# Netflix/metaflow

Hardware: AMD Instinct MI355X
Metric: tokens/sec (higher is better)
Workload: dtype bf16; 1 GPU; model=llama3-8b, global_batch=8, seq_len=4096, parallelism=dp1

## Files before the change

metaflow_amd/ops/csrc/attention.hip:

```cpp

#include "common.h"

#define ATT_D 128

typedef __attribute__((ext_vector_type(16))) float f16f;

DEV f16f mfma32(bf16x8 a, bf16x8 b, f16f c) {
  return __builtin_amdgcn_mfma_f32_32x32x16_bf16(a, b, c, 0, 0, 0);
}

struct WaveCoord {
  int wid, lane, l32, hi;
};

DEV WaveCoord wave_coord() {
  WaveCoord c;
  c.wid = threadIdx.x / WAVE;
  c.lane = threadIdx.x & (WAVE - 1);
  c.l32 = c.lane & 31;
  c.hi = c.lane >> 5;
  return c;
}

DEV int c_row(int r, int hi) { return (r & 3) + 8 * (r >> 2) + 4 * hi; }

DEV unsigned int pack_bf2(float lo, float hi) {
  union { __hip_bfloat162 h; unsigned int u; } c;
  c.h = __float22bfloat162_rn(make_float2(lo, hi));
  return c.u;
}

template <int NT>
DEV void col_to_afrags(const f16f* st, bf16x8* pa, int hi) {
  unsigned int pk[NT * 8], xp[NT * 8];
#pragma unroll
  for (int t = 0; t < NT; ++t)
#pragma unroll
    for (int j2 = 0; j2 < 8; ++j2)
      pk[t * 8 + j2] = pack_bf2(st[t][j2 * 2], st[t][j2 * 2 + 1]);
#pragma unroll
  for (int i = 0; i < NT * 8; ++i) xp[i] = __shfl_xor(pk[i], 32, WAVE);
#pragma unroll
  for (int ks = 0; ks < NT * 2; ++ks) {
    union {
      unsigned int w[4];
      bf16x8 v;
    } u;
    if (hi == 0) {
      u.w[0] = pk[4 * ks];
      u.w[1] = pk[4 * ks + 1];
      u.w[2] = xp[4 * ks];
      u.w[3] = xp[4 * ks + 1];
    } else {
      u.w[0] = xp[4 * ks + 2];
      u.w[1] = xp[4 * ks + 3];
      u.w[2] = pk[4 * ks + 2];
      u.w[3] = pk[4 * ks + 3];
    }
    pa[ks] = u.v;
  }
}


template <int ROWS, int BLOCK>
DEV void stage_panel(short* dst, const short* src,
                     long long src_row_stride) {
  constexpr int TOT = ROWS * 16;
#pragma unroll
  for (int it = 0; it < (TOT + BLOCK - 1) / BLOCK; ++it) {
    const int idx = it * BLOCK + threadIdx.x;
    if (idx < TOT) {
      const int r = idx % ROWS, c8 = idx / ROWS;
      bf16x8 v = *(const bf16x8*)(src + r * src_row_stride + c8 * 8);
      *(bf16x8*)(dst + (c8 >> 1) * (ROWS * 16) + r * 16 + (c8 & 1) * 8) =
          v;
    }
  }
}

template <int ROWS>
DEV bf16x8 frag8_panel(const short* tile, int row, int d0) {
  return *(const bf16x8*)(tile + (d0 >> 4) * (ROWS * 16) + row * 16
                          + (d0 & 15));
}

DEV unsigned long long tr_read(const short* lds_ptr) {
  unsigned int addr = (unsigned int)(unsigned long long)lds_ptr;
  unsigned long long out;
  asm volatile("ds_read_b64_tr_b16 %0, %1" : "=v"(out) : "v"(addr));
  return out;
}

union BFrag {
  unsigned long long u[2];
  bf16x8 v;
};

template <int ROWS>
DEV void tr_load_bfrags(BFrag bfr[4], const short* tile, int row0,
                        int lane, int hi) {
  const int tr_lane_off = (((lane >> 2) & 3) * 16) + (lane & 3) * 4;
  const int tr_panel = ((lane >> 4) & 1) * (ROWS * 16);
#pragma unroll
  for (int n = 0; n < 4; ++n) {
    const int base = n * 2 * (ROWS * 16) + tr_panel
                     + (row0 + hi * 8) * 16 + tr_lane_off;
    bfr[n].u[0] = tr_read(tile + base);
    bfr[n].u[1] = tr_read(tile + base + 4 * 16);
  }
}

DEV void put_elem(short* p, float x) { *p = f2bf(x); }
DEV void put_elem(float* p, float x) { *p = x; }

template <bool ROW_SCALE, typename T>
DEV void store_acc_tile(T* dst, long long off0, int row0, const f16f acc[4],
                        int l32, int hi, float lane_scale = 1.f) {
#pragma unroll
  for (int r = 0; r < 16; ++r) {
    const int row_local = c_row(r, hi);
    float f = 1.f;
    if (ROW_SCALE) f = __shfl(lane_scale, row_local + 32 * hi, WAVE);
    const long long obase = off0 + (long long)(row0 + row_local) * ATT_D;
#pragma unroll
    for (int n = 0; n < 4; ++n)
      put_elem(dst + obase + n * 32 + l32,
               ROW_SCALE ? acc[n][r] * f : acc[n][r]);
  }
}

DEV void acc_to_bfrags(const f16f& x, bf16x8* pb) {
#pragma unroll
  for (int s = 0; s < 2; ++s) {
    unsigned int w[4];
#pragma unroll
    for (int i = 0; i < 4; ++i)
      w[i] = pack_bf2(x[8 * s + 2 * i], x[8 * s + 2 * i + 1]);
    union {
      unsigned int w[4];
      bf16x8 v;
    } u;
#pragma unroll
    for (int i = 0; i < 2; ++i) {
      auto r = __builtin_amdgcn_permlane32_swap(w[i], w[2 + i], false,
                                                false);
      u.w[i] = r[0];
      u.w[2 + i] = r[1];
    }
    pb[s] = u.v;
  }
}

DEV float half_pair_max(float x) {
  const unsigned int u = __float_as_uint(x);
  auto r = __builtin_amdgcn_permlane32_swap(u, u, false, false);
  return fmaxf(__uint_as_float(r[0]), __uint_as_float(r[1]));
}

DEV float half_pair_sum(float x) {
  const unsigned int u = __float_as_uint(x);
  auto r = __builtin_amdgcn_permlane32_swap(u, u, false, false);
  return __uint_as_float(r[0]) + __uint_as_float(r[1]);
}

DEV void lds_wave_fence() {
  __builtin_amdgcn_fence(__ATOMIC_RELEASE, "wavefront");
  __builtin_amdgcn_wave_barrier();
  __builtin_amdgcn_fence(__ATOMIC_ACQUIRE, "wavefront");
}

template <int NB, bool ROW_SCALE>
DEV void store_acc_tile_t_bf16(short* dst, long long off0, short* tw,
                               const f16f acc[4], int lane,
                               float lane_scale = 1.f) {
  constexpr int SLOTS = NB * 4;
  constexpr int ROWLEN = NB * 32;
  const int l32 = lane & 31, hi = lane >> 5;
#pragma unroll
  for (int p = 0; p < 4 / NB; ++p) {
#pragma unroll
    for (int nb = 0; nb < NB; ++nb) {
      const int n = p * NB + nb;
#pragma unroll
      for (int g = 0; g < 4; ++g) {
        bf16x4 w;
#pragma unroll
        for (int j = 0; j < 4; ++j)
          w[j] = f2bf(ROW_SCALE ? acc[n][4 * g + j] * lane_scale
                                : acc[n][4 * g + j]);
        const int slot = (nb * 4 + g) ^ (l32 & (SLOTS - 1));
        *(bf16x4*)(tw + l32 * ROWLEN + slot * 8 + hi * 4) = w;
      }
    }
    lds_wave_fence();
#pragma unroll
    for (int i = 0; i < SLOTS / 2; ++i) {
      const int row = i * (64 / SLOTS) + lane / SLOTS;
      const int c = lane & (SLOTS - 1);
      const bf16x8 v = *(const bf16x8*)(tw + row * ROWLEN
                                        + ((c ^ (row & (SLOTS - 1))) * 8));
      *(bf16x8*)(dst + off0 + (long long)row * ATT_D + p * ROWLEN + c * 8) =
          v;
    }
    if (p + 1 < 4 / NB) lds_wave_fence();
  }
}

struct BlockCoord {
  int rank, h, b;
};

DEV BlockCoord block_coord(int T, int H) {
  const int bid = blockIdx.x;
  const int per_b = T * H;
  BlockCoord c;
  c.b = bid / per_b;
  const int r = bid - c.b * per_b;
  c.rank = r / H;
  c.h = r - c.rank * H;
  return c;
}


template <int BLOCK>
__global__ __launch_bounds__(512) void attn_fwd_v2_kernel(
    const short* __restrict__ q, const short* __restrict__ k,
    const short* __restrict__ v, short* __restrict__ o,
    float* __restrict__ lse, int B, int H, int Hkv, int S, float scale,
    int causal) {
  constexpr int BQ = 256, BKV = 64;
  __shared__ short kp[2][BKV * ATT_D];
  __shared__ short vp[2][BKV * ATT_D];

  const BlockCoord bc = block_coord(S / BQ, H);
  const int qb = S / BQ - 1 - bc.rank;
  const int h = bc.h;
  const int b = bc.b;
  const int hk = h / (H / Hkv);
  const WaveCoord c = wave_coord();
  const int wid = c.wid, lane = c.lane, l32 = c.l32, hi = c.hi;

  const int my_qrow = qb * BQ + wid * 32 + l32;
  const long long hoff = ((long long)b * H + h) * S;
  const long long qoff = (hoff + qb * BQ) * ATT_D;
  const long long kvoff0 = ((long long)b * Hkv + hk) * S * ATT_D;

  bf16x8 q_reg[8];
  {
    const short* qrow = q + (hoff + my_qrow) * ATT_D;
#pragma unroll
    for (int s = 0; s < 8; ++s)
      q_reg[s] = *(const bf16x8*)(qrow + s * 16 + hi * 8);
  }

  float m_run = -INFINITY;
  float l_run = 0.f;
  f16f acc_o[4];
#pragma unroll
  for (int n = 0; n < 4; ++n) acc_o[n] = (f16f){};

  const int tid = threadIdx.x;
  bf16x8 stg_k[2], stg_v[2];
  int stg_r[2], stg_c8[2];
#pragma unroll
  for (int u = 0; u < 2; ++u) {
    const int idx = u * BLOCK + tid;
    stg_r[u] = idx / 16;
    stg_c8[u] = idx % 16;
  }

#define MFX_STAGE_LOAD(jj)                                               \
  {                                                                      \
    const short* kb_ = k + kvoff0 + (long long)(jj) * BKV * ATT_D;       \
    const short* vb_ = v + kvoff0 + (long long)(jj) * BKV * ATT_D;       \
    _Pragma("unroll") for (int u = 0; u < 2; ++u) {                      \
      stg_k[u] = *(const bf16x8*)(kb_ + stg_r[u] * ATT_D + stg_c8[u] * 8);\
      stg_v[u] = *(const bf16x8*)(vb_ + stg_r[u] * ATT_D + stg_c8[u] * 8);\
    }                                                                    \
  }

#define MFX_STAGE_WRITE(buf)                                             \
  {                                                                      \
    _Pragma("unroll") for (int u = 0; u < 2; ++u) {                      \
      const int pel_ = (stg_c8[u] >> 1) * (BKV * 16) + stg_r[u] * 16     \
                       + (stg_c8[u] & 1) * 8;                            \
      *(bf16x8*)(kp[buf] + pel_) = stg_k[u];                             \
      *(bf16x8*)(vp[buf] + pel_) = stg_v[u];                             \
    }                                                                    \
  }

  const int kv_tiles =
      causal ? (qb * BQ + BQ) / BKV : S / BKV;
  MFX_STAGE_LOAD(0);
  MFX_STAGE_WRITE(0);
  __syncthreads();
  for (int j = 0; j < kv_tiles; ++j) {
    const int cur = j & 1;
    if (j + 1 < kv_tiles) MFX_STAGE_LOAD(j + 1);

    const bool active = !causal || (j * BKV <= qb * BQ + wid * 32 + 31);
    if (active) {

    f16f st[2];
#pragma unroll
    for (int t = 0; t < 2; ++t) {
      st[t] = (f16f){};
#pragma unroll
      for (int s = 0; s < 8; ++s) {
        bf16x8 kf = frag8_panel<BKV>(kp[cur], t * 32 + l32,
                                     s * 16 + hi * 8);
        st[t] = mfma32(kf, q_reg[s], st[t]);
      }
    }

    const bool diag = causal && (j * BKV + BKV > qb * BQ);
    float pmax = -INFINITY;
#pragma unroll
    for (int t = 0; t < 2; ++t) {
#pragma unroll
      for (int r = 0; r < 16; ++r) {
        float sv = st[t][r] * scale;
        if (diag) {
          const int kvg = j * BKV + t * 32 + c_row(r, hi);
          if (kvg > my_qrow) sv = -INFINITY;
        }
        st[t][r] = sv;
        pmax = fmaxf(pmax, sv);
      }
    }
    pmax = half_pair_max(pmax);
    const float newm = fmaxf(m_run, pmax);
    const float rescale = __expf(m_run - newm);
    m_run = newm;

    float psum = 0.f;
#pragma unroll
    for (int t = 0; t < 2; ++t)
#pragma unroll
      for (int r = 0; r < 16; ++r) {
        float e = __expf(st[t][r] - newm);
        st[t][r] = e;
        psum += e;
      }
    psum = half_pair_sum(psum);
    l_run = l_run * rescale + psum;

#pragma unroll
    for (int n = 0; n < 4; ++n)
#pragma unroll
      for (int r = 0; r < 16; ++r) acc_o[n][r] *= rescale;

    bf16x8 pb[4];
    acc_to_bfrags(st[0], pb);
    acc_to_bfrags(st[1], pb + 2);

    {
      const int tr_lane_off = (((lane >> 2) & 3) * 16) + (lane & 3) * 4;
      const int tr_panel = ((lane >> 4) & 1) * (BKV * 16);
#pragma unroll
      for (int ks = 0; ks < 4; ++ks) {
        BFrag bfr[4];
#pragma unroll
        for (int n = 0; n < 4; ++n) {
          const int base = n * 2 * (BKV * 16) + tr_panel
                           + (ks * 16 + hi * 8) * 16 + tr_lane_off;
          bfr[n].u[0] = tr_read(vp[cur] + base);
          bfr[n].u[1] = tr_read(vp[cur] + base + 4 * 16);
        }
        asm volatile("s_waitcnt lgkmcnt(0)");
        __builtin_amdgcn_sched_barrier(0);
#pragma unroll
        for (int n = 0; n < 4; ++n)
          acc_o[n] = mfma32(bfr[n].v, pb[ks], acc_o[n]);
      }
    }
    }

    if (j + 1 < kv_tiles) MFX_STAGE_WRITE(cur ^ 1);
    __syncthreads();
  }
#undef MFX_STAGE_LOAD
#undef MFX_STAGE_WRITE

  float inv_l = 1.f / l_run;
  short* tw = (wid < 4 ? &kp[0][0] : &vp[0][0]) + (wid & 3) * (32 * ATT_D);
  store_acc_tile_t_bf16<4, true>(o, qoff + (long long)wid * 32 * ATT_D, tw,
                                 acc_o, lane, inv_l);
  if (hi == 0)
    lse[hoff + my_qrow] = m_run + __logf(l_run);
}

__global__ void attn_bwd_delta_kernel(const short* __restrict__ dout,
                                      const short* __restrict__ o,
                                      float* __restrict__ delta,
                                      long long rows) {
  const int lane = threadIdx.x & (WAVE - 1);
  const int wid = threadIdx.x / WAVE;
  const long long row = (long long)blockIdx.x * (blockDim.x / WAVE) + wid;
  if (row >= rows) return;
  const short* dr = dout + row * ATT_D;
  const short* orow = o + row * ATT_D;
  float s = bf2f(dr[lane]) * bf2f(orow[lane])
            + bf2f(dr[lane + 64]) * bf2f(orow[lane + 64]);
  s = wave_sum(s);
  if (lane == 0) delta[row] = s;
}


extern __shared__ __attribute__((aligned(16))) short dq_kv2[];
#define DQ_DYN_LDS (2 * 64 * ATT_D * 2)

template <int BLOCK>
__global__ __launch_bounds__(512) void attn_bwd_dq_v2_kernel(
    const short* __restrict__ q, const short* __restrict__ k,
    const short* __restrict__ v, const short* __restrict__ dout,
    const float* __restrict__ lse, const float* __restrict__ delta,
    short* __restrict__ dq, int B, int H, int Hkv, int S, float scale,
    int causal) {
  constexpr int BQ = 256, BKV = 64;
  __shared__ short kp[BKV * ATT_D];
  __shared__ short vp[BKV * ATT_D];

  const BlockCoord bc = block_coord(S / BQ, H);
  const int qb = S / BQ - 1 - bc.rank;
  const int h = bc.h;
  const int b = bc.b;
  const int hk = h / (H / Hkv);
  const int wid = threadIdx.x / WAVE;
  const int lane = threadIdx.x & (WAVE - 1);
  const int l32 = lane & 31;
  const int hi = lane >> 5;

  const int my_qrow = qb * BQ + wid * 32 + l32;
  const long long hoff = ((long long)b * H + h) * S;
  const long long qoff = (hoff + qb * BQ) * ATT_D;
  const long long kvoff0 = ((long long)b * Hkv + hk) * S * ATT_D;

  bf16x8 q_reg[8], do_reg[8];
  {
    const short* qrow = q + (hoff + my_qrow) * ATT_D;
    const short* drow = dout + (hoff + my_qrow) * ATT_D;
#pragma unroll
    for (int s = 0; s < 8; ++s) {
      q_reg[s] = *(const bf16x8*)(qrow + s * 16 + hi * 8);
      do_reg[s] = *(const bf16x8*)(drow + s * 16 + hi * 8);
    }
  }
  const float my_lse = lse[hoff + my_qrow];
  const float my_del = delta[hoff + my_qrow];

  f16f acc_dq[4];
#pragma unroll
  for (int n = 0; n < 4; ++n) acc_dq[n] = (f16f){};

  const int tid = threadIdx.x;
  bf16x8 stg_k[2], stg_v[2];
#define MFX_DQ_LOAD(jj)                                                  \
  {                                                                      \
    const short* kb_ = k + kvoff0 + (long long)(jj) * BKV * ATT_D;       \
    const short* vb_ = v + kvoff0 + (long long)(jj) * BKV * ATT_D;       \
    _Pragma("unroll") for (int u = 0; u < 2; ++u) {                      \
      const int idx_ = u * BLOCK + tid;                                  \
      stg_k[u] = *(const bf16x8*)(kb_ + (idx_ / 16) * ATT_D + (idx_ % 16) * 8);\
      stg_v[u] = *(const bf16x8*)(vb_ + (idx_ / 16) * ATT_D + (idx_ % 16) * 8);\
    }                                                                    \
  }
#define MFX_DQ_WRITE(buf)                                                \
  {                                                                      \
    _Pragma("unroll") for (int u = 0; u < 2; ++u) {                      \
      const int idx_ = u * BLOCK + tid;                                  \
      const int pel_ = ((idx_ % 16) >> 1) * (BKV * 16) + (idx_ / 16) * 16\
                       + ((idx_ % 16) & 1) * 8;                          \
      *(bf16x8*)(((buf) ? dq_kv2 : kp) + pel_) = stg_k[u];               \
      *(bf16x8*)(((buf) ? dq_kv2 + BKV * ATT_D : vp) + pel_) = stg_v[u]; \
    }                                                                    \
  }
  const int kv_tiles = causal ? (qb * BQ + BQ) / BKV : S / BKV;
  MFX_DQ_LOAD(0);
  MFX_DQ_WRITE(0);
  __syncthreads();
  for (int j = 0; j < kv_tiles; ++j) {
    const int cur = j & 1;
    const short* kpc = cur ? dq_kv2 : kp;
    const short* vpc = cur ? dq_kv2 + BKV * ATT_D : vp;
    if (j + 1 < kv_tiles) MFX_DQ_LOAD(j + 1);
    if (!(causal && j * BKV > qb * BQ + wid * 32 + 31)) {

#pragma unroll
    for (int t = 0; t < 2; ++t) {
      f16f st = (f16f){}, dpt = (f16f){};
#pragma unroll
      for (int s = 0; s < 8; ++s) {
        bf16x8 kf = frag8_panel<BKV>(kpc, t * 32 + l32, s * 16 + hi * 8);
        bf16x8 vf = frag8_panel<BKV>(vpc, t * 32 + l32, s * 16 + hi * 8);
        st = mfma32(kf, q_reg[s], st);
        dpt = mfma32(vf, do_reg[s], dpt);
      }
#pragma unroll
      for (int r = 0; r < 16; ++r) {
        const int kvg = j * BKV + t * 32 + c_row(r, hi);
        float p = 0.f;
        if (!causal || kvg <= my_qrow)
          p = __expf(st[r] * scale - my_lse);
        st[r] = p * (dpt[r] - my_del) * scale;
      }
      bf16x8 pb[2];
      acc_to_bfrags(st, pb);
#pragma unroll
      for (int ks = 0; ks < 2; ++ks) {
        BFrag bfr[4];
        tr_load_bfrags<BKV>(bfr, kpc, t * 32 + ks * 16, lane, hi);
        asm volatile("s_waitcnt lgkmcnt(0)");
        __builtin_amdgcn_sched_barrier(0);
#pragma unroll
        for (int n = 0; n < 4; ++n)
          acc_dq[n] = mfma32(bfr[n].v, pb[ks], acc_dq[n]);
      }
    }
    }
    if (j + 1 < kv_tiles) MFX_DQ_WRITE(cur ^ 1);
    __syncthreads();
  }
#undef MFX_DQ_LOAD
#undef MFX_DQ_WRITE

  short* tw = (wid < 4 ? kp : vp) + (wid & 3) * (32 * 64);
  store_acc_tile_t_bf16<2, false>(dq, qoff + (long long)wid * 32 * ATT_D,
                                  tw, acc_dq, lane);
}


DEV void store_acc_tile_t(float* dst, long long off0, float* tw,
                          const f16f acc[4], int l32, int hi) {
#pragma unroll
  for (int n = 0; n < 4; ++n) {
#pragma unroll
    for (int r = 0; r < 16; ++r) {
      const int dl = (r & 3) + 8 * (r >> 2) + 4 * hi;
      tw[l32 * 32 + (dl ^ l32)] = acc[n][r];
    }
    lds_wave_fence();
#pragma unroll
    for (int i = 0; i < 16; ++i) {
      const int row = 2 * i + hi;
      dst[off0 + (long long)row * ATT_D + n * 32 + l32] =
          tw[row * 32 + (l32 ^ row)];
    }
    lds_wave_fence();
  }
}

extern __shared__ __attribute__((aligned(16))) short dkdv_v_img[];
#define DKDV_DYN_LDS (256 * ATT_D * 2)

template <int BLOCK>
__global__ __launch_bounds__(512) void attn_bwd_dkdv_v2_kernel(
    const short* __restrict__ q, const short* __restrict__ k,
    const short* __restrict__ v, const short* __restrict__ dout,
    const float* __restrict__ lse, const float* __restrict__ delta,
    float* __restrict__ dk_part, float* __restrict__ dv_part,
    int B, int H, int Hkv, int S, float scale, int causal) {
  constexpr int BKVB = 256, BQ2 = 64;
  __shared__ short qp[BQ2 * ATT_D];
  __shared__ short dop[BQ2 * ATT_D];
  __shared__ float lse_s[BQ2];
  __shared__ float del_s[BQ2];

  const BlockCoord bc = block_coord(S / BKVB, H);
  const int kvb = bc.rank;
  const int h = bc.h;
  const int b = bc.b;
  const int G = H / Hkv;
  const int hk = h / G;
  const int wid = threadIdx.x / WAVE;
  const int lane = threadIdx.x & (WAVE - 1);
  const int l32 = lane & 31;
  const int hi = lane >> 5;

  const int my_kvrow = kvb * BKVB + wid * 32 + l32;
  const long long kvoff =
      (((long long)b * Hkv + hk) * S + kvb * BKVB) * ATT_D;

  bf16x8 kr[8];
  short* vimg = dkdv_v_img + wid * (32 * ATT_D) + lane * 8;
  {
    const short* krow = k + kvoff + (long long)(wid * 32 + l32) * ATT_D;
    const short* vrow = v + kvoff + (long long)(wid * 32 + l32) * ATT_D;
#pragma unroll
    for (int s = 0; s < 8; ++s) {
      kr[s] = *(const bf16x8*)(krow + s * 16 + hi * 8);
      *(bf16x8*)(vimg + s * 512) = *(const bf16x8*)(vrow + s * 16 + hi * 8);
    }
#pragma unroll
    for (int s = 0; s < 8; ++s) asm volatile("" : "+v"(kr[s]));
  }

  f16f acc_dk[4], acc_dv[4];
#pragma unroll
  for (int n = 0; n < 4; ++n) {
    acc_dk[n] = (f16f){};
    acc_dv[n] = (f16f){};
  }

  const long long hoff = ((long long)b * H + h) * S;
  const int jq0 = causal ? (kvb * BKVB) / BQ2 : 0;
  const int nq = S / BQ2;
  for (int jq = jq0; jq < nq; ++jq) {
    __syncthreads();
    const short* qsrc = q + (hoff + (long long)jq * BQ2) * ATT_D;
    const short* dsrc = dout + (hoff + (long long)jq * BQ2) * ATT_D;
    stage_panel<BQ2, BLOCK>(qp, qsrc, ATT_D);
    stage_panel<BQ2, BLOCK>(dop, dsrc, ATT_D);
    if (threadIdx.x < BQ2) {
      lse_s[threadIdx.x] = lse[hoff + jq * BQ2 + threadIdx.x];
      del_s[threadIdx.x] = delta[hoff + jq * BQ2 + threadIdx.x];
    }
    __syncthreads();
    if (causal && jq * BQ2 + BQ2 - 1 < kvb * BKVB + wid * 32) continue;

#pragma unroll
    for (int t = 0; t < 2; ++t) {
      f16f st = (f16f){}, dpt = (f16f){};
#pragma unroll
      for (int s = 0; s < 8; ++s) {
        bf16x8 qf = frag8_panel<BQ2>(qp, t * 32 + l32, s * 16 + hi * 8);
        bf16x8 df = frag8_panel<BQ2>(dop, t * 32 + l32, s * 16 + hi * 8);
        bf16x8 vf = *(const bf16x8*)(vimg + s * 512);
        st = mfma32(qf, kr[s], st);
        dpt = mfma32(df, vf, dpt);
      }
#pragma unroll
      for (int g = 0; g < 4; ++g) {
        const int q0l = t * 32 + g * 8 + 4 * hi;
        const f32x4 lv = *(const f32x4*)&lse_s[q0l];
        const f32x4 dl = *(const f32x4*)&del_s[q0l];
#pragma unroll
        for (int j = 0; j < 4; ++j) {
          const int r = g * 4 + j;
          const int qrg = jq * BQ2 + q0l + j;
          float p = 0.f;
          if (!causal || qrg >= my_kvrow)
            p = __expf(st[r] * scale - lv[j]);
          st[r] = p;
          dpt[r] = p * (dpt[r] - dl[j]) * scale;
        }
      }
      bf16x8 pb[2], pbk[2];
      acc_to_bfrags(st, pb);
      BFrag bfr[2][4];
      const int tr_lane_off = (((lane >> 2) & 3) * 16) + (lane & 3) * 4;
      const int tr_panel = ((lane >> 4) & 1) * (BQ2 * 16);
      const short* g_tile[4] = {dop, dop, qp, qp};
      int g_q0[4];
      g_q0[0] = t * 32;
      g_q0[1] = t * 32 + 16;
      g_q0[2] = t * 32;
      g_q0[3] = t * 32 + 16;
#pragma unroll
      for (int n = 0; n < 4; ++n) {
        const int base = n * 2 * (BQ2 * 16) + tr_panel
                         + (g_q0[0] + hi * 8) * 16 + tr_lane_off;
        bfr[0][n].u[0] = tr_read(g_tile[0] + base);
        bfr[0][n].u[1] = tr_read(g_tile[0] + base + 4 * 16);
      }
      acc_to_bfrags(dpt, pbk);
#pragma unroll
      for (int g = 0; g < 4; ++g) {
        const int cur = g & 1;
        if (g < 3) {
#pragma unroll
          for (int n = 0; n < 4; ++n) {
            const int base = n * 2 * (BQ2 * 16) + tr_panel
                             + (g_q0[g + 1] + hi * 8) * 16 + tr_lane_off;
            bfr[cur ^ 1][n].u[0] = tr_read(g_tile[g + 1] + base);
            bfr[cur ^ 1][n].u[1] = tr_read(g_tile[g + 1] + base + 4 * 16);
          }
          asm volatile("s_waitcnt lgkmcnt(8)");
        } else {
          asm volatile("s_waitcnt lgkmcnt(0)");
        }
        __builtin_amdgcn_sched_barrier(0);
        const bf16x8 bop = (g < 2) ? pb[g] : pbk[g - 2];
        f16f* acc = (g < 2) ? acc_dv : acc_dk;
#pragma unroll
        for (int n = 0; n < 4; ++n)
          acc[n] = mfma32(bfr[cur][n].v, bop, acc[n]);
      }
    }
  }

  __syncthreads();
  float* tw = (float*)(wid < 4 ? qp : dop) + (wid & 3) * 1024;
  const long long poff =
      (hoff + (long long)kvb * BKVB + wid * 32) * ATT_D;
  store_acc_tile_t(dk_part, poff, tw, acc_dk, l32, hi);
  store_acc_tile_t(dv_part, poff, tw, acc_dv, l32, hi);
}

__global__ void dkdv_reduce_kernel(const float* __restrict__ dk_part,
                                   const float* __restrict__ dv_part,
                                   short* __restrict__ dk,
                                   short* __restrict__ dv,
                                   long long n4_kv, int G,
                                   long long head_elems) {
  const long long stride = (long long)gridDim.x * blockDim.x;
  for (long long i4 = (long long)blockIdx.x * blockDim.x + threadIdx.x;
       i4 < n4_kv; i4 += stride) {
    const long long i = i4 * 4;
    const long long slot = i / head_elems;
    const long long rem = i - slot * head_elems;
    const float* kp = dk_part + slot * G * head_elems + rem;
    const float* vp = dv_part + slot * G * head_elems + rem;
    f32x4 ks = *(const f32x4*)kp;
    f32x4 vs = *(const f32x4*)vp;
    for (int g = 1; g < G; ++g) {
      const f32x4 k2 = *(const f32x4*)(kp + (long long)g * head_elems);
      const f32x4 v2 = *(const f32x4*)(vp + (long long)g * head_elems);
#pragma unroll
      for (int j = 0; j < 4; ++j) {
        ks[j] += k2[j];
        vs[j] += v2[j];
      }
    }
    bf16x4 ko, vo;
#pragma unroll
    for (int j = 0; j < 4; ++j) {
      ko[j] = f2bf(ks[j]);
      vo[j] = f2bf(vs[j]);
    }
    *(bf16x4*)(dk + i) = ko;
    *(bf16x4*)(dv + i) = vo;
  }
}
```

metaflow_amd/ops/csrc/debug_kernels.hip:

```cpp

#include "common.h"

typedef __attribute__((ext_vector_type(16))) float f16x_;
__global__ void dbg_mfma32_kernel(const short* __restrict__ a,
                                  const short* __restrict__ b,
                                  float* __restrict__ c ) {
  const int lane = threadIdx.x & 63;
  const int l32 = lane & 31;
  const int hi = lane >> 5;
  bf16x8 av, bv;
#pragma unroll
  for (int i = 0; i < 8; ++i) {
    av[i] = a[l32 * 16 + hi * 8 + i];
    bv[i] = b[(hi * 8 + i) * 32 + l32];
  }
  f16x_ acc = {};
  acc = __builtin_amdgcn_mfma_f32_32x32x16_bf16(av, bv, acc, 0, 0, 0);
#pragma unroll
  for (int r = 0; r < 16; ++r) {
    int row = (r & 3) + 8 * (r >> 2) + 4 * hi;
    c[row * 32 + l32] = acc[r];
  }
}

__global__ __launch_bounds__(64) void dbg_attn_layout_kernel(
    const short* __restrict__ t, const short* __restrict__ x,
    float* __restrict__ st_out, float* __restrict__ o_out) {
  constexpr int ROWS = 64;
  __shared__ short tp[ROWS * ATT_D];
  const WaveCoord c = wave_coord();

  stage_panel<ROWS, WAVE>(tp, t, ATT_D);
  __syncthreads();

  bf16x8 x_reg[8];
#pragma unroll
  for (int s = 0; s < 8; ++s)
    x_reg[s] = *(const bf16x8*)(x + c.l32 * ATT_D + s * 16 + c.hi * 8);

  f16f st[2];
#pragma unroll
  for (int u = 0; u < 2; ++u) {
    st[u] = (f16f){};
#pragma unroll
    for (int s = 0; s < 8; ++s)
      st[u] = mfma32(frag8_panel<ROWS>(tp, u * 32 + c.l32,
                                       s * 16 + c.hi * 8),
                     x_reg[s], st[u]);
#pragma unroll
    for (int r = 0; r < 16; ++r)
      st_out[(u * 32 + c_row(r, c.hi)) * 32 + c.l32] = st[u][r];
  }

  bf16x8 pa[4];
  col_to_afrags<2>(st, pa, c.hi);

  f16f acc[4];
#pragma unroll
  for (int n = 0; n < 4; ++n) acc[n] = (f16f){};
#pragma unroll
  for (int ks = 0; ks < 4; ++ks) {
    BFrag bfr[4];
    tr_load_bfrags<ROWS>(bfr, tp, ks * 16, c.lane, c.hi);
    asm volatile("s_waitcnt lgkmcnt(0)");
    __builtin_amdgcn_sched_barrier(0);
#pragma unroll
    for (int n = 0; n < 4; ++n) acc[n] = mfma32(pa[ks], bfr[n].v, acc[n]);
  }
  store_acc_tile<false>(o_out, 0, 0, acc, c.l32, c.hi);
}
```

metaflow_amd/ops/csrc/mfx_hip.hip:

```cpp

#include <torch/extension.h>
#include <hip/hip_runtime.h>
#include <c10/hip/HIPStream.h>

#include <vector>

#include "elementwise.hip"
#include "adam.hip"
#include "cross_entropy.hip"
#include "attention.hip"
#include "paged.hip"
#include "decode.hip"
#include "append.hip"
#include "debug_kernels.hip"

namespace {

constexpr int kBlock = 256;
constexpr int kGridCap = 2048;

inline hipStream_t cur_stream() {
  return c10::hip::getCurrentHIPStream().stream();
}

// ... 490 lines not shown
          splits, (float)scale);
    else
      attn_append_kernel<NW><<<grid, NW * WAVE, 0, cur_stream()>>>(
          bf(q), bf(kc), bf(vc), pos.data_ptr<int>(), bfm(o), o_part_p,
          ml_part_p, B, H, Hkv, Sq, Lmax, splits, (float)scale);
  };
  if (plan.small)
    launch(std::integral_constant<int, 1>{});
  else
    launch(std::integral_constant<int, 4>{});
  HIP_CHECK_KERNEL();
  if (splits > 1) {
    const long long R = (long long)B * H * Sq;
    attn_append_merge_kernel<<<(int)((R + 3) / 4), 256, 0, cur_stream()>>>(
        o_part_p, ml_part_p, bfm(o), R, splits);
    HIP_CHECK_KERNEL();
  }
  return o;
}

torch::Tensor attn_append(torch::Tensor q, torch::Tensor kc,
                          torch::Tensor vc, torch::Tensor pos,
                          long max_len, double scale) {
  check_bf16(q, "q");
  check_bf16(kc, "kc");
  check_bf16(vc, "vc");
  TORCH_CHECK(q.dim() == 4 && q.size(3) == 128 && q.size(2) >= 1,
              "append expects q [B,H,Sq,128]");
  const int B = q.size(0), H = q.size(1);
  TORCH_CHECK(kc.dim() == 4 && kc.size(0) == B && kc.size(3) == 128,
              "append expects k_cache [B,Hkv,Lmax,128]");
  TORCH_CHECK(vc.sizes() == kc.sizes(),
              "k_cache and v_cache must have the same shape");
  const int Hkv = kc.size(1), Lmax = kc.size(2);
  TORCH_CHECK(H % Hkv == 0, "GQA requires H % Hkv == 0");
  TORCH_CHECK(max_len >= 1 && max_len <= Lmax,
              "max_len must be in [1, Lmax]");
  check_int32_vec(pos, B, "pos");
  return append_launch(q, kc, vc, nullptr, pos, Hkv, Lmax, 0, 0, max_len,
                       scale);
}

void check_page_pool(const torch::Tensor& kp, const torch::Tensor& vp) {
  check_bf16(kp, "k_pages");
  check_bf16(vp, "v_pages");
  TORCH_CHECK(kp.dim() == 4 && kp.size(2) == PG_ROWS && kp.size(3) == PG_D,
              "page pool must be [num_pages, Hkv, 64, 128]");
  TORCH_CHECK(vp.sizes() == kp.sizes(),
              "k_pages and v_pages must have the same shape");
}

void check_block_table(const torch::Tensor& table, int B) {
  TORCH_CHECK(table.is_cuda() && table.scalar_type() == torch::kInt32 &&
              table.dim() == 2 && table.size(0) == B &&
              table.is_contiguous(),
              "block_table must be contiguous int32 [B, pages_per_seq] "
              "on GPU");
}

torch::Tensor attn_decode_paged(torch::Tensor q, torch::Tensor kp,
                                torch::Tensor vp, torch::Tensor table,
                                torch::Tensor lengths, long max_len,
                                double scale) {
  check_bf16(q, "q");
  check_page_pool(kp, vp);
  TORCH_CHECK(q.dim() == 4 && q.size(2) == 1 && q.size(3) == PG_D,
              "paged decode expects q [B,H,1,128]");
  const int B = q.size(0), H = q.size(1);
  const int num_pages = kp.size(0), Hkv = kp.size(1);
  TORCH_CHECK(H % Hkv == 0, "GQA requires H % Hkv == 0");
  check_block_table(table, B);
  const int table_stride = table.size(1);
  TORCH_CHECK(max_len >= 1 && max_len <= (long)table_stride * PG_ROWS,
              "max_len must be in [1, 64 * pages_per_seq]");
  check_int32_vec(lengths, B, "lengths");
  const int splits = (int)std::min<long>(
      decode_splits(B, H, max_len), (max_len + PG_ROWS - 1) / PG_ROWS);
  return decode_launch(q, kp, vp, table.data_ptr<int>(), lengths, Hkv, 0,
                       num_pages, table_stride, splits, scale);
}

torch::Tensor attn_append_paged(torch::Tensor q, torch::Tensor kp,
                                torch::Tensor vp, torch::Tensor table,
                                torch::Tensor pos, long max_len,
                                double scale) {
  check_bf16(q, "q");
  check_page_pool(kp, vp);
  TORCH_CHECK(q.dim() == 4 && q.size(3) == PG_D && q.size(2) >= 1,
              "paged append expects q [B,H,Sq,128]");
  const int B = q.size(0), H = q.size(1);
  const int num_pages = kp.size(0), Hkv = kp.size(1);
  TORCH_CHECK(H % Hkv == 0, "GQA requires H % Hkv == 0");
  check_block_table(table, B);
  const int table_stride = table.size(1);
  TORCH_CHECK(max_len >= 1 && max_len <= (long)table_stride * PG_ROWS,
              "max_len must be in [1, 64 * pages_per_seq]");
  check_int32_vec(pos, B, "pos");
  return append_launch(q, kp, vp, table.data_ptr<int>(), pos, Hkv, 0,
                       num_pages, table_stride, max_len, scale);
}

void check_new_rows(const torch::Tensor& t, const char* name) {
  TORCH_CHECK(t.is_cuda() && t.scalar_type() == torch::kBFloat16,
              name, " must be bf16 on GPU");
  TORCH_CHECK(t.dim() == 4 && t.size(3) == PG_D && t.stride(3) == 1,
              name, " must be [B,Hkv,S,128] with a dense last dim");
  TORCH_CHECK(t.stride(0) % 8 == 0 && t.stride(1) % 8 == 0 &&
              t.stride(2) % 8 == 0 &&
              reinterpret_cast<uintptr_t>(t.data_ptr()) % 16 == 0,
              name, " rows must be 16-byte aligned");
}

void kv_page_write(torch::Tensor k, torch::Tensor v, torch::Tensor kp,
                   torch::Tensor vp, torch::Tensor table,
                   torch::Tensor pos) {
  check_new_rows(k, "k");
  check_new_rows(v, "v");
  check_page_pool(kp, vp);
  TORCH_CHECK(v.sizes() == k.sizes(), "k and v must have the same shape");
  const int B = k.size(0), Hkv = k.size(1), S = k.size(2);
  TORCH_CHECK(kp.size(1) == Hkv, "k and the pool disagree on Hkv");
  check_block_table(table, B);
  check_int32_vec(pos, B, "pos");
  const long long vecs = (long long)B * Hkv * S * (PG_D / 8);
  if (vecs == 0) return;
  kv_page_write_kernel<<<grid_for(vecs), kBlock, 0, cur_stream()>>>(
      bf(k), bf(v), bfm(kp), bfm(vp), table.data_ptr<int>(),
      pos.data_ptr<int>(), B, Hkv, S, (int)kp.size(0), (int)table.size(1),
      k.stride(0), k.stride(1), k.stride(2), v.stride(0), v.stride(1),
      v.stride(2));
  HIP_CHECK_KERNEL();
}

torch::Tensor dbg_mfma32(torch::Tensor a, torch::Tensor b) {
  auto out = torch::empty({32, 32}, a.options().dtype(torch::kFloat32));
  dbg_mfma32_kernel<<<1, 64, 0, cur_stream()>>>(bf(a), bf(b),
                                                out.data_ptr<float>());
  HIP_CHECK_KERNEL();
  return out;
}

std::vector<torch::Tensor> dbg_attn_layout(torch::Tensor t,
                                           torch::Tensor x) {
  check_bf16(t, "t");
  check_bf16(x, "x");
  TORCH_CHECK(t.dim() == 2 && t.size(0) == 64 && t.size(1) == 128,
              "t must be [64,128]");
  TORCH_CHECK(x.dim() == 2 && x.size(0) == 32 && x.size(1) == 128,
              "x must be [32,128]");
  auto f32opts = t.options().dtype(torch::kFloat32);
  auto st = torch::empty({64, 32}, f32opts);
  auto out = torch::empty({32, 128}, f32opts);
  dbg_attn_layout_kernel<<<1, 64, 0, cur_stream()>>>(
      bf(t), bf(x), st.data_ptr<float>(), out.data_ptr<float>());
  HIP_CHECK_KERNEL();
  return {st, out};
}

}

PYBIND11_MODULE(TORCH_EXTENSION_NAME, m) {
  m.def("rmsnorm_fwd", &rmsnorm_fwd, "RMSNorm forward (bf16)");
  m.def("rmsnorm_bwd", &rmsnorm_bwd, "RMSNorm backward");
  m.def("add_rmsnorm_fwd", &add_rmsnorm_fwd, "fused residual add + RMSNorm");
  m.def("rope", &rope, "RoPE (half-rotation), fwd or bwd via sign");
  m.def("swiglu_fwd", &swiglu_fwd, "SwiGLU forward");
  m.def("swiglu_bwd", &swiglu_bwd, "SwiGLU backward");
  m.def("swiglu_gu_fwd", [](torch::Tensor gu){ return swiglu_gu_fwd(gu)[0]; }, "fused-layout SwiGLU fwd");
  m.def("swiglu_gu_bwd", &swiglu_gu_bwd, "fused-layout SwiGLU bwd");
  m.def("add_bf16", &add_bf16, "fused bf16 add");
  m.def("decode_tokens_u16", &decode_tokens_u16,
        "packed uint16 token bytes -> int64 tokens (one pass on-GPU)");
  m.def("quant_e5m2", &quant_e5m2,
        "bf16 -> OCP E5M2 bytes, one fused scale+saturate+convert pass "
        "(v_cvt_pk_bf8_f32; for delayed-scaled GRADIENT quantization)");
  m.def("quant_e4m3", &quant_e4m3,
        "one-pass bf16 -> OCP E4M3 (uint8 storage) with scale");
  m.def("adamw", &adamw, "fused AdamW (bf16 p/g, fp32 m/v[, master])");
  m.def("cross_entropy_fwd", &cross_entropy_fwd, "fused CE forward");
  m.def("cross_entropy_bwd", &cross_entropy_bwd, "fused CE backward");
  m.def("rope_qkv_fwd", &rope_qkv_fwd,
        "fused QKV split + transpose + RoPE");
  m.def("rope_qkv_bwd", &rope_qkv_bwd,
        "fused QKV rope backward -> GEMM-grad layout");
  m.def("attn_fwd", &attn_fwd, "flash attention forward (causal, GQA)");
  m.def("attn_bwd", &attn_bwd, "flash attention backward");
  m.def("attn_decode", &attn_decode,
        "split-K flash-decode over the KV cache (q [B,H,1,128])");
  m.def("attn_decode_varlen", &attn_decode_varlen,
        "flash-decode with per-sequence cache lengths (int32 [B]; "
        "length 0 = inactive slot, output 0)");
  m.def("attn_append", &attn_append,
        "append attention: Sq query rows at per-sequence offsets pos "
        "(int32 [B]) over the KV cache (q [B,H,Sq,128])");
  m.def("attn_decode_paged", &attn_decode_paged,
        "flash-decode over a paged KV cache: pool [P,Hkv,64,128], block "
        "table int32 [B,pages], lengths int32 [B] (0 = output 0)");
  m.def("attn_append_paged", &attn_append_paged,
        "append attention over a paged KV cache: q [B,H,Sq,128], pool "
        "[P,Hkv,64,128], block table int32 [B,pages], pos int32 [B] "
        "(pos < 0 = output 0)");
  m.def("kv_page_write", &kv_page_write,
        "scatter new K/V rows [B,Hkv,S,128] into the page pool at "
        "pos[b].. through the block table (pos < 0 skips the sequence)");
  m.def("dbg_mfma32", &dbg_mfma32, "mfma 32x32x16 layout probe");
  m.def("dbg_attn_layout", &dbg_attn_layout,
        "attention panel / transposed-read / col_to_afrags layout probe");
}
```

Before: 21840 tokens/s.

## Switch attention LDS tiles to a swizzled dual-use image with immediate-offset reads

Replaces the panel LDS layout for K/V (forward and dQ) and Q/dO (dK/dV backward) with a swizzled image layout whose addresses reduce to a per-lane base plus compile-time immediates. Both row fragment reads and ds_read_b64_tr_b16 transposed reads can then use offset fields instead of per-iteration address arithmetic, and the XOR swizzle is meant to cut LDS bank conflicts. Causal masking is also restructured so the mask loop runs only on diagonal or edge tiles, using a wave-uniform check. A debug probe kernel is added to validate the new layout. Correctness depends on the hand-derived swizzle maps matching the MFMA and transpose-read lane patterns.

```diff
diff --git a/metaflow_amd/ops/csrc/attention.hip b/metaflow_amd/ops/csrc/attention.hip
--- a/metaflow_amd/ops/csrc/attention.hip
+++ b/metaflow_amd/ops/csrc/attention.hip
@@ -1,5 +1,6 @@
 
 #include "common.h"
+#include "attn_lds_image.h"
 
 #define ATT_D 128
 
@@ -110,6 +111,49 @@
   }
 }
 
+
+DEV unsigned int lds_addr(const void* p) {
+  return (unsigned int)(unsigned long long)p;
+}
+
+DEV unsigned long long tr_read_imm(unsigned int base, int imm) {
+  unsigned long long out;
+  asm volatile("ds_read_b64_tr_b16 %0, %1 offset:%2"
+               : "=v"(out)
+               : "v"(base), "i"(imm));
+  return out;
+}
+
+DEV bf16x8 img_row_frag(const short* tile, int rb0, int rb1, int t, int s) {
+  return *(const bf16x8*)((const char*)tile + ((s & 1) ? rb1 : rb0)
+                          + lds_img::row_imm_a(t, s));
+}
+
+DEV void img_tr_load(BFrag bfr[4], unsigned int tb0, unsigned int tb1,
+                     int ks) {
+#pragma unroll
+  for (int n = 0; n < 4; ++n) {
+    bfr[n].u[0] = tr_read_imm(tb0, lds_img::tr_imm_a(ks, n));
+    bfr[n].u[1] = tr_read_imm(tb1, lds_img::tr_imm_a(ks, n));
+  }
+}
+
+template <int ROWS, int BLOCK>
+DEV void stage_image(short* dst, const short* src,
+                     long long src_row_stride) {
+  constexpr int TOT = ROWS * 16;
+#pragma unroll
+  for (int it = 0; it < (TOT + BLOCK - 1) / BLOCK; ++it) {
+    const int idx = it * BLOCK + threadIdx.x;
+    if (idx < TOT) {
+      const int r = lds_img::stage_walk_row(ROWS, idx);
+      const int ch = lds_img::stage_walk_ch(ROWS, idx);
+      bf16x8 v = *(const bf16x8*)(src + r * src_row_stride + ch * 8);
+      *(bf16x8*)((char*)dst + lds_img::off_a(r, ch)) = v;
+    }
+  }
+}
+
 DEV void put_elem(short* p, float x) { *p = f2bf(x); }
 DEV void put_elem(float* p, float x) { *p = x; }
 
@@ -265,9 +309,14 @@
 #pragma unroll
   for (int u = 0; u < 2; ++u) {
     const int idx = u * BLOCK + tid;
-    stg_r[u] = idx / 16;
-    stg_c8[u] = idx % 16;
-  }
+    stg_r[u] = lds_img::stage16_row(idx);
+    stg_c8[u] = lds_img::stage16_ch(idx);
+  }
+  const int stg_off = lds_img::stage16_addr_a(tid);
+  const int rb0 = lds_img::row_base_a(lane, 0);
+  const int rb1 = lds_img::row_base_a(lane, 1);
+  const unsigned int tb0 = lds_addr(&vp[0][0]) + lds_img::tr_base_a(lane, 0);
+  const unsigned int tb1 = lds_addr(&vp[0][0]) + lds_img::tr_base_a(lane, 1);
 
 #define MFX_STAGE_LOAD(jj)                                               \
   {                                                                      \
@@ -282,10 +331,9 @@
 #define MFX_STAGE_WRITE(buf)                                             \
   {                                                                      \
     _Pragma("unroll") for (int u = 0; u < 2; ++u) {                      \
-      const int pel_ = (stg_c8[u] >> 1) * (BKV * 16) + stg_r[u] * 16     \
-                       + (stg_c8[u] & 1) * 8;                            \
-      *(bf16x8*)(kp[buf] + pel_) = stg_k[u];                             \
-      *(bf16x8*)(vp[buf] + pel_) = stg_v[u];                             \
+      const int pel_ = stg_off + u * 8192;                               \
+      *(bf16x8*)((char*)kp[buf] + pel_) = stg_k[u];                      \
+      *(bf16x8*)((char*)vp[buf] + pel_) = stg_v[u];                      \
     }                                                                    \
   }
 
@@ -307,27 +355,30 @@
       st[t] = (f16f){};
 #pragma unroll
       for (int s = 0; s < 8; ++s) {
-        bf16x8 kf = frag8_panel<BKV>(kp[cur], t * 32 + l32,
-                                     s * 16 + hi * 8);
+        bf16x8 kf = img_row_frag(kp[cur], rb0, rb1, t, s);
         st[t] = mfma32(kf, q_reg[s], st[t]);
       }
     }
 
     const bool diag = causal && (j * BKV + BKV > qb * BQ);
+#pragma unroll
+    for (int t = 0; t < 2; ++t)
+#pragma unroll
+      for (int r = 0; r < 16; ++r) st[t][r] *= scale;
+    if (diag) {
+#pragma unroll
+      for (int t = 0; t < 2; ++t)
+#pragma unroll
+        for (int r = 0; r < 16; ++r) {
+          const int kvg = j * BKV + t * 32 + c_row(r, hi);
+          if (kvg > my_qrow) st[t][r] = -INFINITY;
+        }
+    }
     float pmax = -INFINITY;
 #pragma unroll
-    for (int t = 0; t < 2; ++t) {
-#pragma unroll
-      for (int r = 0; r < 16; ++r) {
-        float sv = st[t][r] * scale;
-        if (diag) {
-          const int kvg = j * BKV + t * 32 + c_row(r, hi);
-          if (kvg > my_qrow) sv = -INFINITY;
-        }
-        st[t][r] = sv;
-        pmax = fmaxf(pmax, sv);
-      }
-    }
+    for (int t = 0; t < 2; ++t)
+#pragma unroll
+      for (int r = 0; r < 16; ++r) pmax = fmaxf(pmax, st[t][r]);
     pmax = half_pair_max(pmax);
     const float newm = fmaxf(m_run, pmax);
     const float rescale = __expf(m_run - newm);
@@ -355,18 +406,12 @@
     acc_to_bfrags(st[1], pb + 2);
 
     {
-      const int tr_lane_off = (((lane >> 2) & 3) * 16) + (lane & 3) * 4;
-      const int tr_panel = ((lane >> 4) & 1) * (BKV * 16);
+      const unsigned int tbc0 = tb0 + cur * (BKV * ATT_D * 2);
+      const unsigned int tbc1 = tb1 + cur * (BKV * ATT_D * 2);
 #pragma unroll
       for (int ks = 0; ks < 4; ++ks) {
         BFrag bfr[4];
-#pragma unroll
-        for (int n = 0; n < 4; ++n) {
-          const int base = n * 2 * (BKV * 16) + tr_panel
-                           + (ks * 16 + hi * 8) * 16 + tr_lane_off;
-          bfr[n].u[0] = tr_read(vp[cur] + base);
-          bfr[n].u[1] = tr_read(vp[cur] + base + 4 * 16);
-        }
+        img_tr_load(bfr, tbc0, tbc1, ks);
         asm volatile("s_waitcnt lgkmcnt(0)");
         __builtin_amdgcn_sched_barrier(0);
 #pragma unroll
@@ -455,6 +500,12 @@
 
   const int tid = threadIdx.x;
   bf16x8 stg_k[2], stg_v[2];
+  const int stg_off = lds_img::stage16_addr_a(tid);
+  const int rb0 = lds_img::row_base_a(lane, 0);
+  const int rb1 = lds_img::row_base_a(lane, 1);
+  const int trl0 = lds_img::tr_base_a(lane, 0);
+  const int trl1 = lds_img::tr_base_a(lane, 1);
+  const int wid_s = __builtin_amdgcn_readfirstlane(threadIdx.x) / WAVE;
 #define MFX_DQ_LOAD(jj)                                                  \
   {                                                                      \
     const short* kb_ = k + kvoff0 + (long long)(jj) * BKV * ATT_D;       \
@@ -468,11 +519,10 @@
 #define MFX_DQ_WRITE(buf)                                                \
   {                                                                      \
     _Pragma("unroll") for (int u = 0; u < 2; ++u) {                      \
-      const int idx_ = u * BLOCK + tid;                                  \
-      const int pel_ = ((idx_ % 16) >> 1) * (BKV * 16) + (idx_ / 16) * 16\
-                       + ((idx_ % 16) & 1) * 8;                          \
-      *(bf16x8*)(((buf) ? dq_kv2 : kp) + pel_) = stg_k[u];               \
-      *(bf16x8*)(((buf) ? dq_kv2 + BKV * ATT_D : vp) + pel_) = stg_v[u]; \
+      const int pel_ = stg_off + u * 8192;                               \
+      *(bf16x8*)((char*)((buf) ? dq_kv2 : kp) + pel_) = stg_k[u];        \
+      *(bf16x8*)((char*)((buf) ? dq_kv2 + BKV * ATT_D : vp) + pel_) =    \
+          stg_v[u];                                                      \
     }                                                                    \
   }
   const int kv_tiles = causal ? (qb * BQ + BQ) / BKV : S / BKV;
@@ -491,25 +541,30 @@
       f16f st = (f16f){}, dpt = (f16f){};
 #pragma unroll
       for (int s = 0; s < 8; ++s) {
-        bf16x8 kf = frag8_panel<BKV>(kpc, t * 32 + l32, s * 16 + hi * 8);
-        bf16x8 vf = frag8_panel<BKV>(vpc, t * 32 + l32, s * 16 + hi * 8);
+        bf16x8 kf = img_row_frag(kpc, rb0, rb1, t, s);
+        bf16x8 vf = img_row_frag(vpc, rb0, rb1, t, s);
         st = mfma32(kf, q_reg[s], st);
         dpt = mfma32(vf, do_reg[s], dpt);
       }
 #pragma unroll
-      for (int r = 0; r < 16; ++r) {
-        const int kvg = j * BKV + t * 32 + c_row(r, hi);
-        float p = 0.f;
-        if (!causal || kvg <= my_qrow)
-          p = __expf(st[r] * scale - my_lse);
-        st[r] = p * (dpt[r] - my_del) * scale;
-      }
+      for (int r = 0; r < 16; ++r) st[r] = __expf(st[r] * scale - my_lse);
+      if (causal && j * BKV + t * 32 + 31 > qb * BQ + wid_s * 32) {
+#pragma unroll
+        for (int r = 0; r < 16; ++r) {
+          const int kvg = j * BKV + t * 32 + c_row(r, hi);
+          if (kvg > my_qrow) st[r] = 0.f;
+        }
+      }
+#pragma unroll
+      for (int r = 0; r < 16; ++r)
+        st[r] = st[r] * (dpt[r] - my_del) * scale;
       bf16x8 pb[2];
       acc_to_bfrags(st, pb);
 #pragma unroll
       for (int ks = 0; ks < 2; ++ks) {
         BFrag bfr[4];
-        tr_load_bfrags<BKV>(bfr, kpc, t * 32 + ks * 16, lane, hi);
+        img_tr_load(bfr, lds_addr(kpc) + trl0, lds_addr(kpc) + trl1,
+                    t * 2 + ks);
         asm volatile("s_waitcnt lgkmcnt(0)");
         __builtin_amdgcn_sched_barrier(0);
 #pragma unroll
@@ -561,8 +616,9 @@
     float* __restrict__ dk_part, float* __restrict__ dv_part,
     int B, int H, int Hkv, int S, float scale, int causal) {
   constexpr int BKVB = 256, BQ2 = 64;
-  __shared__ short qp[BQ2 * ATT_D];
-  __shared__ short dop[BQ2 * ATT_D];
+  __shared__ short qdo[2 * BQ2 * ATT_D];
+  short* const qp = qdo;
+  short* const dop = qdo + BQ2 * ATT_D;
   __shared__ float lse_s[BQ2];
   __shared__ float del_s[BQ2];
 
@@ -602,6 +658,13 @@
     acc_dv[n] = (f16f){};
   }
 
+  const int rb0 = lds_img::row_base_a(lane, 0);
+  const int rb1 = lds_img::row_base_a(lane, 1);
+  const unsigned int tb0 = lds_addr(qp) + lds_img::tr_base_a(lane, 0);
+  const unsigned int tb1 = lds_addr(qp) + lds_img::tr_base_a(lane, 1);
+  constexpr int DOP_REL = BQ2 * ATT_D * 2;
+  const int wid_s = __builtin_amdgcn_readfirstlane(threadIdx.x) / WAVE;
+
   const long long hoff = ((long long)b * H + h) * S;
   const int jq0 = causal ? (kvb * BKVB) / BQ2 : 0;
   const int nq = S / BQ2;
@@ -609,8 +672,8 @@
     __syncthreads();
     const short* qsrc = q + (hoff + (long long)jq * BQ2) * ATT_D;
     const short* dsrc = dout + (hoff + (long long)jq * BQ2) * ATT_D;
-    stage_panel<BQ2, BLOCK>(qp, qsrc, ATT_D);
-    stage_panel<BQ2, BLOCK>(dop, dsrc, ATT_D);
+    stage_image<BQ2, BLOCK>(qp, qsrc, ATT_D);
+    stage_image<BQ2, BLOCK>(dop, dsrc, ATT_D);
     if (threadIdx.x < BQ2) {
       lse_s[threadIdx.x] = lse[hoff + jq * BQ2 + threadIdx.x];
       del_s[threadIdx.x] = delta[hoff + jq * BQ2 + threadIdx.x];
@@ -623,57 +686,56 @@
       f16f st = (f16f){}, dpt = (f16f){};
 #pragma unroll
       for (int s = 0; s < 8; ++s) {
-        bf16x8 qf = frag8_panel<BQ2>(qp, t * 32 + l32, s * 16 + hi * 8);
-        bf16x8 df = frag8_panel<BQ2>(dop, t * 32 + l32, s * 16 + hi * 8);
+        bf16x8 qf = img_row_frag(qp, rb0, rb1, t, s);
+        bf16x8 df = img_row_frag(dop, rb0, rb1, t, s);
         bf16x8 vf = *(const bf16x8*)(vimg + s * 512);
         st = mfma32(qf, kr[s], st);
         dpt = mfma32(df, vf, dpt);
       }
+      const bool edge =
+          causal && jq * BQ2 + t * 32 < kvb * BKVB + wid_s * 32 + 31;
 #pragma unroll
       for (int g = 0; g < 4; ++g) {
         const int q0l = t * 32 + g * 8 + 4 * hi;
         const f32x4 lv = *(const f32x4*)&lse_s[q0l];
         const f32x4 dl = *(const f32x4*)&del_s[q0l];
+        float p[4];
+#pragma unroll
+        for (int j = 0; j < 4; ++j)
+          p[j] = __expf(st[g * 4 + j] * scale - lv[j]);
+        if (edge) {
+          asm volatile("");
+#pragma unroll
+          for (int j = 0; j < 4; ++j)
+            if (jq * BQ2 + q0l + j < my_kvrow) p[j] = 0.f;
+        }
 #pragma unroll
         for (int j = 0; j < 4; ++j) {
           const int r = g * 4 + j;
-          const int qrg = jq * BQ2 + q0l + j;
-          float p = 0.f;
-          if (!causal || qrg >= my_kvrow)
-            p = __expf(st[r] * scale - lv[j]);
-          st[r] = p;
-          dpt[r] = p * (dpt[r] - dl[j]) * scale;
+          st[r] = p[j];
+          dpt[r] = p[j] * (dpt[r] - dl[j]) * scale;
         }
       }
       bf16x8 pb[2], pbk[2];
       acc_to_bfrags(st, pb);
       BFrag bfr[2][4];
-      const int tr_lane_off = (((lane >> 2) & 3) * 16) + (lane & 3) * 4;
-      const int tr_panel = ((lane >> 4) & 1) * (BQ2 * 16);
-      const short* g_tile[4] = {dop, dop, qp, qp};
-      int g_q0[4];
-      g_q0[0] = t * 32;
-      g_q0[1] = t * 32 + 16;
-      g_q0[2] = t * 32;
-      g_q0[3] = t * 32 + 16;
 #pragma unroll
       for (int n = 0; n < 4; ++n) {
-        const int base = n * 2 * (BQ2 * 16) + tr_panel
-                         + (g_q0[0] + hi * 8) * 16 + tr_lane_off;
-        bfr[0][n].u[0] = tr_read(g_tile[0] + base);
-        bfr[0][n].u[1] = tr_read(g_tile[0] + base + 4 * 16);
+        const int imm = DOP_REL + lds_img::tr_imm_a(2 * t, n);
+        bfr[0][n].u[0] = tr_read_imm(tb0, imm);
+        bfr[0][n].u[1] = tr_read_imm(tb1, imm);
       }
       acc_to_bfrags(dpt, pbk);
 #pragma unroll
       for (int g = 0; g < 4; ++g) {
         const int cur = g & 1;
         if (g < 3) {
+          const int rel = (g + 1 < 2) ? DOP_REL : 0;
 #pragma unroll
           for (int n = 0; n < 4; ++n) {
-            const int base = n * 2 * (BQ2 * 16) + tr_panel
-                             + (g_q0[g + 1] + hi * 8) * 16 + tr_lane_off;
-            bfr[cur ^ 1][n].u[0] = tr_read(g_tile[g + 1] + base);
-            bfr[cur ^ 1][n].u[1] = tr_read(g_tile[g + 1] + base + 4 * 16);
+            const int imm = rel + lds_img::tr_imm_a(2 * t + ((g + 1) & 1), n);
+            bfr[cur ^ 1][n].u[0] = tr_read_imm(tb0, imm);
+            bfr[cur ^ 1][n].u[1] = tr_read_imm(tb1, imm);
           }
           asm volatile("s_waitcnt lgkmcnt(8)");
         } else {
diff --git a/metaflow_amd/ops/csrc/attn_lds_image.h b/metaflow_amd/ops/csrc/attn_lds_image.h
--- /dev/null
+++ b/metaflow_amd/ops/csrc/attn_lds_image.h
@@ -0,0 +1,53 @@
+#pragma once
+
+#if defined(__HIPCC__) || defined(__CUDACC__)
+#define LDSIMG_FN __host__ __device__ constexpr
+#else
+#define LDSIMG_FN constexpr
+#endif
+
+namespace lds_img {
+
+LDSIMG_FN int off_a(int row, int ch) {
+  return 2048 * (row >> 3) + 512 * (ch >> 2) + 64 * (row & 7)
+         + 16 * ((ch & 3) ^ ((row >> 2) & 3));
+}
+
+LDSIMG_FN int off_b(int row, int ch) {
+  return 256 * row + 16 * (ch ^ (((row & 3) << 2) | ((row >> 2) & 3)));
+}
+
+LDSIMG_FN int off_panel(int rows, int row, int ch) {
+  return (ch >> 1) * rows * 32 + row * 32 + (ch & 1) * 16;
+}
+
+LDSIMG_FN int row_base_a(int lane, int s_odd) {
+  return off_a(lane & 31, 2 * s_odd + (lane >> 5));
+}
+LDSIMG_FN int row_imm_a(int t, int s) { return 8192 * t + 512 * (s >> 1); }
+LDSIMG_FN int row_addr_a(int lane, int t, int s) {
+  return row_base_a(lane, s & 1) + row_imm_a(t, s);
+}
+
+LDSIMG_FN int tr_base_a(int lane, int u) {
+  return off_a(8 * (lane >> 5) + 4 * u + ((lane >> 2) & 3),
+               2 * ((lane >> 4) & 1) + ((lane & 3) >> 1))
+         + 8 * (lane & 1);
+}
+LDSIMG_FN int tr_imm_a(int ks, int n) { return 4096 * ks + 512 * n; }
+LDSIMG_FN int tr_addr_a(int lane, int ks, int n, int u) {
+  return tr_base_a(lane, u) + tr_imm_a(ks, n);
+}
+
+LDSIMG_FN int stage16_row(int idx) { return idx >> 4; }
+LDSIMG_FN int stage16_ch(int idx) { return idx & 15; }
+LDSIMG_FN int stage16_addr_a(int idx) {
+  return off_a(stage16_row(idx), stage16_ch(idx));
+}
+LDSIMG_FN int stage_walk_row(int rows, int idx) { return idx % rows; }
+LDSIMG_FN int stage_walk_ch(int rows, int idx) { return idx / rows; }
+LDSIMG_FN int stage_walk_addr_a(int rows, int idx) {
+  return off_a(stage_walk_row(rows, idx), stage_walk_ch(rows, idx));
+}
+
+}
diff --git a/metaflow_amd/ops/csrc/debug_kernels.hip b/metaflow_amd/ops/csrc/debug_kernels.hip
--- a/metaflow_amd/ops/csrc/debug_kernels.hip
+++ b/metaflow_amd/ops/csrc/debug_kernels.hip
@@ -69,3 +69,57 @@
   }
   store_acc_tile<false>(o_out, 0, 0, acc, c.l32, c.hi);
 }
+
+__global__ __launch_bounds__(64) void dbg_attn_image_kernel(
+    const short* __restrict__ t, const short* __restrict__ x,
+    float* __restrict__ st_out, float* __restrict__ o_out) {
+  constexpr int ROWS = 64;
+  __shared__ short tp[ROWS * ATT_D];
+  const WaveCoord c = wave_coord();
+
+  stage_image<ROWS, WAVE>(tp, t, ATT_D);
+  __syncthreads();
+
+  bf16x8 x_reg[8];
+#pragma unroll
+  for (int s = 0; s < 8; ++s)
+    x_reg[s] = *(const bf16x8*)(x + c.l32 * ATT_D + s * 16 + c.hi * 8);
+
+  const int rb0 = lds_img::row_base_a(c.lane, 0);
+  const int rb1 = lds_img::row_base_a(c.lane, 1);
+  f16f st[2];
+#pragma unroll
+  for (int u = 0; u < 2; ++u) {
+    st[u] = (f16f){};
+#pragma unroll
+    for (int s = 0; s < 8; ++s)
+      st[u] = mfma32(img_row_frag(tp, rb0, rb1, u, s), x_reg[s], st[u]);
+#pragma unroll
+    for (int r = 0; r < 16; ++r)
+      st_out[(u * 32 + c_row(r, c.hi)) * 32 + c.l32] = st[u][r];
+  }
+
+  bf16x8 pb[4];
+  acc_to_bfrags(st[0], pb);
+  acc_to_bfrags(st[1], pb + 2);
+
+  const unsigned int tb0 = lds_addr(tp) + lds_img::tr_base_a(c.lane, 0);
+  const unsigned int tb1 = lds_addr(tp) + lds_img::tr_base_a(c.lane, 1);
+  f16f acc[4];
+#pragma unroll
+  for (int n = 0; n < 4; ++n) acc[n] = (f16f){};
+#pragma unroll
+  for (int ks = 0; ks < 4; ++ks) {
+    BFrag bfr[4];
+    img_tr_load(bfr, tb0, tb1, ks);
+    asm volatile("s_waitcnt lgkmcnt(0)");
+    __builtin_amdgcn_sched_barrier(0);
+#pragma unroll
+    for (int n = 0; n < 4; ++n) acc[n] = mfma32(bfr[n].v, pb[ks], acc[n]);
+  }
+#pragma unroll
+  for (int n = 0; n < 4; ++n)
+#pragma unroll
+    for (int r = 0; r < 16; ++r)
+      o_out[c.l32 * ATT_D + n * 32 + c_row(r, c.hi)] = acc[n][r];
+}
diff --git a/metaflow_amd/ops/csrc/mfx_hip.hip b/metaflow_amd/ops/csrc/mfx_hip.hip
--- a/metaflow_amd/ops/csrc/mfx_hip.hip
+++ b/metaflow_amd/ops/csrc/mfx_hip.hip
@@ -666,6 +666,23 @@
   auto st = torch::empty({64, 32}, f32opts);
   auto out = torch::empty({32, 128}, f32opts);
   dbg_attn_layout_kernel<<<1, 64, 0, cur_stream()>>>(
+      bf(t), bf(x), st.data_ptr<float>(), out.data_ptr<float>());
+  HIP_CHECK_KERNEL();
+  return {st, out};
+}
+
+std::vector<torch::Tensor> dbg_attn_image(torch::Tensor t,
+                                          torch::Tensor x) {
+  check_bf16(t, "t");
+  check_bf16(x, "x");
+  TORCH_CHECK(t.dim() == 2 && t.size(0) == 64 && t.size(1) == 128,
+              "t must be [64,128]");
+  TORCH_CHECK(x.dim() == 2 && x.size(0) == 32 && x.size(1) == 128,
+              "x must be [32,128]");
+  auto f32opts = t.options().dtype(torch::kFloat32);
+  auto st = torch::empty({64, 32}, f32opts);
+  auto out = torch::empty({32, 128}, f32opts);
+  dbg_attn_image_kernel<<<1, 64, 0, cur_stream()>>>(
       bf(t), bf(x), st.data_ptr<float>(), out.data_ptr<float>());
   HIP_CHECK_KERNEL();
   return {st, out};
@@ -720,4 +737,7 @@
   m.def("dbg_mfma32", &dbg_mfma32, "mfma 32x32x16 layout probe");
   m.def("dbg_attn_layout", &dbg_attn_layout,
         "attention panel / transposed-read / col_to_afrags layout probe");
-}
+  m.def("dbg_attn_image", &dbg_attn_image,
+        "train kernels' dual-use LDS image: staging / row-read / "
+        "transposed-read probe");
+}
```

Result: faster. 22170 tokens/s (median of 6 runs) (+1.5%).
